# spaceml-org/STARCOP

Measured on AMD Instinct MI355X. Metric: 512x512 hyperspectral tiles/sec (train fwd+bwd), higher is better.
Workload: dtype f32; 1 GPU; configs[1]: HyperSTARCOP U-Net (smp.Unet mobilenet_v2, 4ch mag1c+RGB) train step fwd+loss+bwd+Adam, 512x512 tiles, fp32 HIP kernels (3x3 convs: fp32 operands split exactly into 16-bit terms on the matrix cores, fp32 accumulation; see config.precision and DESIGN.md section 2); batch_per_gpu=16, global_batch=16, parallelism=dp1, hipgraph=False, precision=fp32

## Files before the change

starcop_amd/csrc/conv_mfma.hip:

```cpp
#include "sc_common.h"
#include <vector>
#include <cstdlib>

namespace {

struct ConvP {
  SrcD s0, s1;
  const float* wpk;
  int N, H, W, Cout;
  float* out0; float* out1;
  int csplit, accum0, accum1;
  const float* add0; const float* add1;
  float* stats;
  int xcdmap;
};

template <int KS, int RM, bool BNB, int PF_ = 1>
__global__ __launch_bounds__(256, 2) void k_conv_mfma(const ConvP p) {
  constexpr int TAPS = KS * KS;
  constexpr int CO_T = 32 * RM;
  constexpr int PR = (KS == 3) ? 6 : 4;
  constexpr int PC = (KS == 3) ? 34 : 32;
  constexpr int PCH = PR * PC;
  constexpr int KC = (KS == 3) ? 8 : 16;
// ... 327 lines not shown
  const int lane = tid & 63, wave = tid >> 6;
  const int l15 = lane & 15, lq = lane >> 4;
  const int n = blockIdx.z;
  const int H = p.H, W = p.W;
  const int tiles_x = (W + 31) >> 5;
  const int ty = blockIdx.x / tiles_x;
  const int y0 = ty * 4 * RW, x0 = (blockIdx.x - ty * tiles_x) * 32;
  const int C0 = p.s0.C;
  const int Cin = C0 + p.s1.C;
  const int nk = (Cin + KC - 1) / KC;
  const float* wbase = p.wpk;

  floatx4 acc[RW][2];
#pragma unroll
  for (int rr = 0; rr < RW; ++rr) { acc[rr][0] = (floatx4){0.f, 0.f, 0.f, 0.f}; acc[rr][1] = acc[rr][0]; }

  const int sci = tid >> 5, sq = tid & 31;
  unsigned off0[NE], off1[NE];
  unsigned inb = 0;
  {
    const int up0 = p.s0.up, up1 = p.s1.up;
    const int Ws0 = W >> up0, Ws1 = W >> up1;
#pragma unroll
    for (int i = 0; i < NE; ++i) {
      const int e = sq + 32 * i;
      const int pr = e / PC, pc = e - pr * PC;
      const int y = y0 - 1 + pr, x = x0 - 1 + pc;
      const bool ok = (e < PCH) && (y >= 0) && (y < H) && (x >= 0) && (x < W);
      off0[i] = ok ? (unsigned)((y >> up0) * Ws0 + (x >> up0)) : 0u;
      off1[i] = ok ? (unsigned)((y >> up1) * Ws1 + (x >> up1)) : 0u;
      inb |= ok ? (1u << i) : 0u;
    }
  }
  float xv[NE], av[BNB ? NE : 1];
  float4 c0 = make_float4(1.f, 0.f, 0.f, 0.f);
  float c4 = 0.f, slo = 0.f, shi = 0.f;
  bool chok = true;
  floatx4 wv[NW];

  auto load_chunk = [&](int kc) {
    const int cg = kc * KC + sci;
    const bool second = cg >= C0;
    const SrcD& s = second ? p.s1 : p.s0;
    chok = cg < Cin;
    const int cs = chok ? (second ? cg - C0 : cg) : 0;
    slo = sc_act_lo(s.act); shi = sc_act_hi(s.act);
    if (s.mode != SC_SRC_RAW) { c0 = *reinterpret_cast<const float4*>(s.cst + (size_t)cs * SC_CST); c4 = BNB ? s.cst[(size_t)cs * SC_CST + 4] : 0.f; }
    else { c0 = make_float4(1.f, 0.f, 0.f, 0.f); c4 = 0.f; }
    const size_t plane = (size_t)(H >> s.up) * (W >> s.up);
    const float* xb = s.x + ((size_t)n * s.C + cs) * plane;
    const float* ab = BNB ? s.aux + ((size_t)n * s.C + cs) * plane : nullptr;
#pragma unroll
    for (int i = 0; i < NE; ++i) {
      const unsigned o = second ? off1[i] : off0[i];
      xv[i] = xb[o];
      if (BNB) av[i] = ab[o];
    }
    const floatx4* wsrc = reinterpret_cast<const floatx4*>(wbase + (size_t)kc * WCH);
#pragma unroll
    for (int j = 0; j < NW; ++j) {
      const int i4 = tid + 256 * j;
      wv[j] = wsrc[i4 < WCH / 4 ? i4 : WCH / 4 - 1];
    }
  };
  auto store_chunk = [&](int buf) {
#pragma unroll
    for (int i = 0; i < NE; ++i) {
      const float t = BNB ? sc_pro_bnbwd(xv[i], av[BNB ? i : 0], c0.x, c0.y, c0.z, c0.w, c4, slo, shi) : sc_pro_affine(xv[i], c0.x, c0.y, slo, shi);
      s_p[buf][sci * PCHP + sq + 32 * i] = (((inb >> i) & 1u) && chok) ? t : 0.f;
    }
#pragma unroll
    for (int j = 0; j < NW; ++j) *reinterpret_cast<floatx4*>(&s_w[buf][(tid + 256 * j) * 4]) = wv[j];
  };
  auto compute_chunk = [&](int buf) {
#pragma unroll
    for (int kq = 0; kq < KC / 4; ++kq) {
      const int cil = 4 * kq + lq;
#pragma unroll
      for (int tap = 0; tap < TAPS; ++tap) {
        const int kh = tap / 3, kw = tap - 3 * kh;
        const float a = s_w[buf][(cil * TAPS + tap) * CO_T + l15];
#pragma unroll
        for (int rr = 0; rr < RW; ++rr)
#pragma unroll
          for (int pb = 0; pb < 2; ++pb) {
            const float b = s_p[buf][cil * PCHP + (wave * RW + rr + kh) * PC + pb * 16 + l15 + kw];
            acc[rr][pb] = __builtin_amdgcn_mfma_f32_16x16x4f32(a, b, acc[rr][pb], 0, 0, 0);
          }
      }
    }
  };

  load_chunk(0);
  store_chunk(0);
  __syncthreads();
  for (int kc = 0; kc < nk; ++kc) {
    const bool more = (kc + 1) < nk;
    if (more) load_chunk(kc + 1);
    compute_chunk(kc & 1);
    if (more) store_chunk((kc + 1) & 1);
    __syncthreads();
  }

  const size_t HWs = (size_t)H * W;
  const bool want_stats = p.stats != nullptr;
#pragma unroll
  for (int r = 0; r < 4; ++r) {
    const int co = 4 * lq + r;
    float s = 0.f, ss = 0.f;
#pragma unroll
    for (int rr = 0; rr < RW; ++rr) {
      const int oy = y0 + wave * RW + rr;
#pragma unroll
      for (int pb = 0; pb < 2; ++pb) {
        const int ox = x0 + pb * 16 + l15;
        float v = acc[rr][pb][r];
        const bool ok = (oy < H) && (ox < W) && (co < p.Cout);
        if (!ok) v = 0.f;
        s += v; ss = fmaf(v, v, ss);
        if (ok) {
          const size_t idx = ((size_t)n * p.Cout + co) * HWs + (size_t)oy * W + ox;
          if (p.add0) v += p.add0[idx];
          if (p.add1) v += p.add1[idx];
          if (p.accum0) v += p.out0[idx];
          p.out0[idx] = v;
        }
      }
    }
    if (want_stats) {
      SC_DPP_ADD(s, 0xB1, 0xF); SC_DPP_ADD(s, 0x4E, 0xF); SC_DPP_ADD(s, 0x141, 0xF); SC_DPP_ADD(s, 0x140, 0xF);
      SC_DPP_ADD(ss, 0xB1, 0xF); SC_DPP_ADD(ss, 0x4E, 0xF); SC_DPP_ADD(ss, 0x141, 0xF); SC_DPP_ADD(ss, 0x140, 0xF);
      if (l15 == 0) { s_red[wave][co][0] = s; s_red[wave][co][1] = ss; }
    }
  }
  if (want_stats) {
    __syncthreads();
    const int rows4 = (H + 3) >> 2;
    const int tx = blockIdx.x - ty * tiles_x;
    for (int i = tid; i < RW * CO_T * 2; i += 256) {
      const int hh = i / (CO_T * 2), rem = i - hh * (CO_T * 2);
      const int co = rem >> 1, k2 = rem & 1;
      const int t4 = RW * ty + hh;
      if (co < p.Cout && t4 < rows4) {
        float t = 0.f;
#pragma unroll
        for (int w2 = 0; w2 < 4 / RW; ++w2) t += s_red[hh * (4 / RW) + w2][co][k2];
        const size_t row = ((size_t)n * rows4 + t4) * tiles_x + tx;
        p.stats[(row * p.Cout + co) * 2 + k2] = t;
      }
    }
  }
}

template <int RM, bool BNB>
__global__ __launch_bounds__(256, 2) void k_conv1_ksplit(const ConvP p) {
  constexpr int CO_T = 32 * RM, KC = 16, PS = 33;
  __shared__ float s_acc[4][CO_T * PS];
  const int tid = threadIdx.x, lane = tid & 63, wave = tid >> 6;
  const int l31 = lane & 31, lhi = lane >> 5;
  const int n = blockIdx.z, cot = blockIdx.y;
  const int HW = p.H * p.W;
  const int p0 = blockIdx.x * 32;
  const int Cin = p.s0.C;
  const int nk = (Cin + KC - 1) / KC;
  const float* wbase = p.wpk + (size_t)cot * nk * KC * CO_T;
  const int pix = p0 + l31;
  const bool pok = pix < HW;
  const float* xb = p.s0.x + (size_t)n * Cin * HW + (pok ? pix : 0);
  const float* ab = BNB ? p.s0.aux + (size_t)n * Cin * HW + (pok ? pix : 0) : nullptr;
  const float* cst = p.s0.cst;
  const float lo = sc_act_lo(p.s0.act), hi = sc_act_hi(p.s0.act);

  floatx16 acc[RM];
#pragma unroll
  for (int m = 0; m < RM; ++m)
#pragma unroll
    for (int r = 0; r < 16; ++r) acc[m][r] = 0.f;

  float bx[8], by[BNB ? 8 : 1], wa[8][RM];
  float4 c0[8]; float c4[BNB ? 8 : 1];
  auto load_chunk = [&](int kc) {
#pragma unroll
    for (int cp = 0; cp < 8; ++cp) {
      const int ci = kc * KC + 2 * cp + lhi;
      const int cc = ci < Cin ? ci : 0;
      bx[cp] = xb[(size_t)cc * HW];
      if (BNB) by[cp] = ab[(size_t)cc * HW];
      if (BNB) { c0[cp] = *reinterpret_cast<const float4*>(cst + (size_t)cc * SC_CST); c4[cp] = cst[(size_t)cc * SC_CST + 4]; }
      else { const float2 t = *reinterpret_cast<const float2*>(cst + (size_t)cc * SC_CST); c0[cp] = make_float4(t.x, t.y, 0.f, 0.f); }
#pragma unroll
      for (int m = 0; m < RM; ++m) wa[cp][m] = wbase[(size_t)ci * CO_T + m * 32 + l31];
    }
  };
  int kc = wave;
  if (kc < nk) load_chunk(kc);
  while (kc < nk) {
    float b[8], a[8][RM];
#pragma unroll
    for (int cp = 0; cp < 8; ++cp) {
      const int ci = kc * KC + 2 * cp + lhi;
      const float t = BNB ? sc_pro_bnbwd(bx[cp], by[BNB ? cp : 0], c0[cp].x, c0[cp].y, c0[cp].z, c0[cp].w, c4[BNB ? cp : 0], lo, hi)
                          : sc_pro_affine(bx[cp], c0[cp].x, c0[cp].y, lo, hi);
      b[cp] = (pok && ci < Cin) ? t : 0.f;
#pragma unroll
      for (int m = 0; m < RM; ++m) a[cp][m] = wa[cp][m];
    }
    const int kn = kc + 4;
    load_chunk(kn < nk ? kn : kc);
#pragma unroll
    for (int cp = 0; cp < 8; ++cp)
#pragma unroll
      for (int m = 0; m < RM; ++m) acc[m] = __builtin_amdgcn_mfma_f32_32x32x2f32(a[cp][m], b[cp], acc[m], 0, 0, 0);
    kc = kn;
  }
#pragma unroll
  for (int m = 0; m < RM; ++m)
#pragma unroll
    for (int r = 0; r < 16; ++r) s_acc[wave][(m * 32 + (r & 3) + 8 * (r >> 2) + 4 * lhi) * PS + l31] = acc[m][r];
  __syncthreads();
  const int px = tid & 31, cg = tid >> 5;
  const int opix = p0 + px;
  const bool ok_px = opix < HW;
  const size_t HWs = (size_t)HW;
  const size_t srow = (size_t)n * gridDim.x + blockIdx.x;
  const bool single = p.csplit == p.Cout;
  const size_t cbase = ((size_t)n * p.Cout + (size_t)cot * CO_T) * HWs;
  float* const ob = p.out0 + cbase;
  const float* const a0 = p.add0 ? p.add0 + cbase : nullptr;
  const float* const a1 = p.add1 ? p.add1 + cbase : nullptr;
#pragma unroll
  for (int i = 0; i < CO_T / 8; ++i) {
    const int col = cg + 8 * i;
    const int co = cot * CO_T + col;
    float v = s_acc[0][col * PS + px] + s_acc[1][col * PS + px] + s_acc[2][col * PS + px] + s_acc[3][col * PS + px];
    const bool ok = ok_px && (co < p.Cout);
    if (!ok) v = 0.f;
    if (p.stats) {
      const float s = half_sum32(v), ss = half_sum32(v * v);
      if ((lane & 31) == SC_HALF_SUM_LANE && co < p.Cout) {
        p.stats[(srow * p.Cout + co) * 2] = s;
        p.stats[(srow * p.Cout + co) * 2 + 1] = ss;
      }
    }
    if (ok) {
      if (single) {
        const unsigned off = (unsigned)col * (unsigned)HWs + (unsigned)opix;
        if (a0) v += a0[off];
        if (a1) v += a1[off];
        if (p.accum0) v += ob[off];
        ob[off] = v;
        continue;
      }
      float* o; size_t idx; int accum;
      if (co < p.csplit) {
        idx = ((size_t)n * p.csplit + co) * HWs + opix; o = p.out0; accum = p.accum0;
      } else {
        idx = ((size_t)n * (p.Cout - p.csplit) + (co - p.csplit)) * HWs + opix; o = p.out1; accum = p.accum1;
      }
      if (p.add0) v += p.add0[idx];
      if (p.add1) v += p.add1[idx];
      if (accum) v += o[idx];
      o[idx] = v;
    }
  }
}

#ifndef SC_PWS_PD
#define SC_PWS_PD 8
#endif
struct PwsP {
  const float* x; const float* aux; const float* cst; int act;
  const float* wpk; int co_t, Kpad;
  float* out; float* stats;
  int HW, K, M;
};

template <int NCB, int NKS, int CP, bool BNB = false>
__global__ __launch_bounds__(256) void k_pw_stream(const PwsP p) {
  constexpr int PD = NKS < SC_PWS_PD ? NKS : SC_PWS_PD;
  constexpr int NPG = 4 / CP;
  constexpr int CW = BNB ? 8 : 2;
  __shared__ __attribute__((aligned(16))) float s_cst[NKS * 4 * CW];
  __shared__ float s_red[4][NCB * 16][2];
  const int tid = threadIdx.x, lane = tid & 63, wave = __builtin_amdgcn_readfirstlane(tid >> 6);
  const int n16 = lane & 15, kq = lane >> 4;
  const int K = p.K, M = p.M, HW = p.HW;
  for (int c = tid; c < NKS * 4; c += 256) {
    if constexpr (BNB) {
      float4 c0 = make_float4(1.f, 0.f, 0.f, 0.f); float c4 = 0.f;
      if (c < K) { c0 = *reinterpret_cast<const float4*>(p.cst + (size_t)c * SC_CST); c4 = p.cst[(size_t)c * SC_CST + 4]; }
      *reinterpret_cast<float4*>(&s_cst[8 * c]) = c0;
      *reinterpret_cast<float4*>(&s_cst[8 * c + 4]) = make_float4(c4, 0.f, 0.f, 0.f);
    } else {
      float sc = 1.f, sh = 0.f;
      if (c < K && p.cst != nullptr) { sc = p.cst[(size_t)c * SC_CST]; sh = p.cst[(size_t)c * SC_CST + 1]; }
      s_cst[2 * c] = sc; s_cst[2 * c + 1] = sh;
    }
  }
  const int pg = wave % NPG, part = wave / NPG;
  const long gpx = ((long)blockIdx.x * NPG + pg) * 64;
  const int img = (int)(gpx / HW), px0 = (int)(gpx - (long)img * HW) + 4 * n16;
  const float* xb = p.x + (size_t)img * K * HW + px0;
  const float* yb = BNB ? p.aux + (size_t)img * K * HW + px0 : nullptr;
  float4 xr[PD], yr[BNB ? PD : 1];
#pragma unroll
  for (int u = 0; u < PD; ++u) {
    const int k = 4 * u + kq;
    xr[u] = *reinterpret_cast<const float4*>(xb + (size_t)(k < K ? k : 0) * HW);
    if constexpr (BNB) yr[u] = *reinterpret_cast<const float4*>(yb + (size_t)(k < K ? k : 0) * HW);
  }
  float A[NCB][NKS];
#pragma unroll
  for (int cb = 0; cb < NCB; ++cb) {
    const int m = (part * NCB + cb) * 16 + n16;
    const float* wp = p.wpk + ((size_t)(m / p.co_t) * p.Kpad) * p.co_t + (m % p.co_t);
#pragma unroll
    for (int ks = 0; ks < NKS; ++ks) {
      const int k = 4 * ks + kq;
      A[cb][ks] = (m < M && k < K) ? wp[(size_t)k * p.co_t] : 0.f;
    }
  }
  floatx4 acc[NCB][4];
#pragma unroll
  for (int cb = 0; cb < NCB; ++cb)
#pragma unroll
    for (int j = 0; j < 4; ++j) acc[cb][j] = (floatx4){0.f, 0.f, 0.f, 0.f};
  const float lo = sc_act_lo(p.act), hi = sc_act_hi(p.act);
  __syncthreads();
#pragma unroll
  for (int ks = 0; ks < NKS; ++ks) {
    const float4 v = xr[ks % PD];
    float4 y = make_float4(0.f, 0.f, 0.f, 0.f);
    if constexpr (BNB) y = yr[ks % PD];
    if (ks + PD < NKS) {
      const int k = 4 * (ks + PD) + kq;
      xr[ks % PD] = *reinterpret_cast<const float4*>(xb + (size_t)(k < K ? k : 0) * HW);
      if constexpr (BNB) yr[ks % PD] = *reinterpret_cast<const float4*>(yb + (size_t)(k < K ? k : 0) * HW);
    }
    float b[4];
    if constexpr (BNB) {
      const float4 c = *reinterpret_cast<const float4*>(&s_cst[8 * (4 * ks + kq)]);
      const float c4 = s_cst[8 * (4 * ks + kq) + 4];
      b[0] = sc_pro_bnbwd(v.x, y.x, c.x, c.y, c.z, c.w, c4, lo, hi); b[1] = sc_pro_bnbwd(v.y, y.y, c.x, c.y, c.z, c.w, c4, lo, hi);
      b[2] = sc_pro_bnbwd(v.z, y.z, c.x, c.y, c.z, c.w, c4, lo, hi); b[3] = sc_pro_bnbwd(v.w, y.w, c.x, c.y, c.z, c.w, c4, lo, hi);
    } else {
      const float2 c = *reinterpret_cast<const float2*>(&s_cst[2 * (4 * ks + kq)]);
      b[0] = sc_pro_affine(v.x, c.x, c.y, lo, hi); b[1] = sc_pro_affine(v.y, c.x, c.y, lo, hi);
      b[2] = sc_pro_affine(v.z, c.x, c.y, lo, hi); b[3] = sc_pro_affine(v.w, c.x, c.y, lo, hi);
    }
#pragma unroll
    for (int cb = 0; cb < NCB; ++cb)
#pragma unroll
      for (int j = 0; j < 4; ++j) acc[cb][j] = __builtin_amdgcn_mfma_f32_16x16x4f32(A[cb][ks], b[j], acc[cb][j], 0, 0, 0);
  }
  float* ob = p.out + (size_t)img * M * HW + px0;
  const bool want_stats = p.stats != nullptr;
#pragma unroll
  for (int cb = 0; cb < NCB; ++cb)
#pragma unroll
    for (int r = 0; r < 4; ++r) {
      const int col = cb * 16 + 4 * kq + r, co = part * NCB * 16 + col;
      const float4 o = make_float4(acc[cb][0][r], acc[cb][1][r], acc[cb][2][r], acc[cb][3][r]);
      if (co < M) *reinterpret_cast<float4*>(ob + (size_t)co * HW) = o;
      if (want_stats) {
        float sv = (o.x + o.y) + (o.z + o.w), sq = fmaf(o.x, o.x, fmaf(o.y, o.y, fmaf(o.z, o.z, o.w * o.w)));
        sv = row_sum16(sv); sq = row_sum16(sq);
        if (n16 == 0) { s_red[wave][col][0] = sv; s_red[wave][col][1] = sq; }
// ... 555 lines not shown
    if (hipMalloc(&d, h.size() * sizeof(float)) != hipSuccess) return nullptr;
    if (hipMemcpy(d, h.data(), h.size() * sizeof(float), hipMemcpyHostToDevice) != hipSuccess) { (void)hipFree(d); return nullptr; }
    table[dev] = d;
  }
  return table[dev];
}

const float* sc_identity_cst_table(int C) { return sc_identity_cst(C); }

extern "C" int sc_pw_stream_variant(const sc_conv_args* a) {
  if (a == nullptr || a->ks != 1 || a->nsrc != 1 || a->N <= 0 || a->H <= 0 || a->W <= 0 || a->Cout <= 0) return -1;
  if (a->co_t != 32 && a->co_t != 64) return -1;
  static const bool pws_off = [] { const char* e = getenv("STARCOP_PWS"); return e && atoi(e) == 0; }();
  const long HWl = (long)a->H * a->W;
  const int K = a->src[0].C, M = a->Cout;
  if (K <= 0 || K % 8 != 0) return -1;
  const bool bnb = a->src[0].mode == SC_SRC_BNBWD;
  if (a->src[0].mode != SC_SRC_RAW && a->src[0].cst == nullptr) return -1;
  if (bnb && a->src[0].aux == nullptr) return -1;
  const bool plain = (a->src[0].mode == SC_SRC_RAW || a->src[0].mode == SC_SRC_AFFINE || (bnb && a->bnr == nullptr && a->stats == nullptr)) &&
                     a->src[0].up == 0 && a->csplit == a->Cout && !a->accum0 && a->add0 == nullptr && a->add1 == nullptr && a->out0 != nullptr;
  const bool aligned = (((uintptr_t)a->src[0].x | (uintptr_t)a->out0 | (bnb ? (uintptr_t)a->src[0].aux : 0)) & 15) == 0;
  const int nks = K / 4;
  const bool ks_ok = bnb ? (nks == 4 || nks == 6 || nks == 8) : (nks == 6 || nks == 8);
  if (pws_off || !plain || !aligned || !ks_ok || M > 192 || HWl < 4096 || HWl % 256 != 0 || HWl >= (1L << 30)) return -1;
  const int ncb = bnb ? (M <= 32 ? 2 : (M <= 96 ? 3 : (M <= 160 ? 5 : 6))) : (M <= 16 ? 1 : (M <= 32 ? 2 : (M <= 160 ? 5 : 6)));
  return (bnb ? 100 : 0) + 10 * ncb + nks;
}

extern "C" int sc_conv2d_mfma(const sc_conv_args* a, sc_stream stream) {
  SC_REQUIRE(a != nullptr, "sc_conv2d_mfma: null args");
  SC_REQUIRE(a->ks == 1 || a->ks == 3, "sc_conv2d_mfma: ks must be 1 or 3 (got %d)", a->ks);
  SC_REQUIRE(a->co_t == 16 || a->co_t == 32 || a->co_t == 64, "sc_conv2d_mfma: co_t must be 16, 32 or 64 (got %d)", a->co_t);
  SC_REQUIRE(a->co_t != 16 || (a->ks == 3 && a->Cout <= 16 && a->csplit == a->Cout),
             "sc_conv2d_mfma: co_t=16 is the thin-layer kernel: ks=3, Cout<=16, single output");
  SC_REQUIRE(a->nsrc == 1 || a->nsrc == 2, "sc_conv2d_mfma: nsrc must be 1 or 2");
  const int C0 = a->src[0].C, C1 = a->nsrc == 2 ? a->src[1].C : 0;
  SC_REQUIRE(C0 > 0 && C0 % 8 == 0 && C1 % 8 == 0, "sc_conv2d_mfma: source channels must be multiples of 8 (got %d,%d)", C0, C1);
  SC_REQUIRE(a->nsrc == 1 || a->ks == 3, "sc_conv2d_mfma: a channel concat of two sources needs ks=3");
  SC_REQUIRE(a->N > 0 && a->H > 0 && a->W > 0 && a->Cout > 0, "sc_conv2d_mfma: bad shape");
  SC_REQUIRE(a->csplit > 0 && a->csplit <= a->Cout, "sc_conv2d_mfma: bad csplit");
  SC_REQUIRE(a->csplit == a->Cout || (a->add0 == nullptr && a->add1 == nullptr), "sc_conv2d_mfma: add tensors need a single output");
  for (int s = 0; s < a->nsrc; ++s) {
    SC_REQUIRE(a->src[s].up == 0 || (a->ks == 3 && a->H % 2 == 0 && a->W % 2 == 0), "sc_conv2d_mfma: upsampled source needs ks=3 and even H,W");
    SC_REQUIRE(a->src[s].mode == SC_SRC_RAW || a->src[s].cst != nullptr, "sc_conv2d_mfma: source %d needs constants", s);
    SC_REQUIRE(a->src[s].mode != SC_SRC_BNBWD || a->src[s].aux != nullptr, "sc_conv2d_mfma: BNBWD source needs aux");
    SC_REQUIRE(a->src[s].mode != SC_SRC_BNBWD || a->nsrc == 1, "sc_conv2d_mfma: a BNBWD source cannot be part of a concat");
  }
  const int pws = a->ks == 1 ? sc_pw_stream_variant(a) : -1;
  if (a->ks == 1) {
    const long HWl = (long)a->H * a->W;
    const int K = a->src[0].C, M = a->Cout;
    if (pws >= 0) {
      const bool bnb = pws >= 100;
      const int ncb = (pws / 10) % 10, nks = pws % 10;
      PwsP q;
      q.x = a->src[0].x; q.aux = a->src[0].aux; q.cst = a->src[0].mode == SC_SRC_RAW ? nullptr : a->src[0].cst;
      q.act = a->src[0].mode == SC_SRC_RAW ? (int)SC_ACT_NONE : a->src[0].act;
      q.wpk = a->wpk; q.co_t = a->co_t; q.Kpad = (K + 15) / 16 * 16;
      q.out = a->out0; q.stats = a->stats; q.HW = (int)HWl; q.K = K; q.M = M;
      hipStream_t st = (hipStream_t)stream;
      const long groups = (long)a->N * HWl / 64;
#define SC_PWS(NCB_, NKS_, CP_) hipLaunchKernelGGL((k_pw_stream<NCB_, NKS_, CP_>), dim3((unsigned)(groups / (4 / CP_))), dim3(256), 0, st, q)
#define SC_PWS_K(NCB_, CP_) do { if (nks == 6) SC_PWS(NCB_, 6, CP_); else SC_PWS(NCB_, 8, CP_); } while (0)
      if (bnb) {
#define SC_PWSB(NCB_, CP_) do { if (nks == 4) hipLaunchKernelGGL((k_pw_stream<NCB_, 4, CP_, true>), dim3((unsigned)(groups / (4 / CP_))), dim3(256), 0, st, q); \
                                else if (nks == 6) hipLaunchKernelGGL((k_pw_stream<NCB_, 6, CP_, true>), dim3((unsigned)(groups / (4 / CP_))), dim3(256), 0, st, q); \
                                else hipLaunchKernelGGL((k_pw_stream<NCB_, 8, CP_, true>), dim3((unsigned)(groups / (4 / CP_))), dim3(256), 0, st, q); } while (0)
        if (ncb == 2) SC_PWSB(2, 1);
        else if (ncb == 3) SC_PWSB(3, 2);
        else if (ncb == 5) SC_PWSB(5, 2);
        else SC_PWSB(6, 2);
#undef SC_PWSB
      }
      else if (ncb == 1) SC_PWS_K(1, 1);
      else if (ncb == 2) SC_PWS_K(2, 1);
      else if (ncb == 5) SC_PWS_K(5, 2);
      else SC_PWS_K(6, 2);
#undef SC_PWS_K
#undef SC_PWS
      SC_LAUNCH_OK("sc_conv2d_mfma(k_pw_stream)");
      return SC_OK;
    }
  }
  ConvP p;
  p.s0 = to_srcd(a->src[0]);
  p.s1 = a->nsrc == 2 ? to_srcd(a->src[1]) : empty_srcd();
  if (a->ks == 1) {
    if (p.s0.mode == SC_SRC_RAW) { p.s0.cst = sc_identity_cst(p.s0.C); SC_REQUIRE(p.s0.cst != nullptr, "sc_conv2d_mfma: identity constants unavailable (C = %d)", p.s0.C); }
    if (a->nsrc == 2 && p.s1.mode == SC_SRC_RAW) { p.s1.cst = sc_identity_cst(p.s1.C); SC_REQUIRE(p.s1.cst != nullptr, "sc_conv2d_mfma: identity constants unavailable (C = %d)", p.s1.C); }
  }
  p.wpk = a->wpk; p.N = a->N; p.H = a->H; p.W = a->W; p.Cout = a->Cout;
  p.out0 = a->out0; p.out1 = a->out1; p.csplit = a->csplit; p.accum0 = a->accum0; p.accum1 = a->accum1;
  p.add0 = a->add0; p.add1 = a->add1; p.stats = a->stats;
  const int co_tiles = (a->Cout + a->co_t - 1) / a->co_t;
  dim3 grid;
  if (a->ks == 3) grid = dim3(((a->W + 31) / 32) * ((a->H + 3) / 4), co_tiles, a->N);
  else grid = dim3((a->H * a->W + 127) / 128, co_tiles, a->N);
  hipStream_t st = (hipStream_t)stream;
  p.xcdmap = 0;
  constexpr int xcdmap_env = 0;
  if (a->co_t != 16 && xcdmap_env) {
    const long total = (long)grid.x * a->N, per_xcd = (total + 7) / 8;
    SC_REQUIRE(per_xcd * 8 * co_tiles < (1L << 31), "sc_conv2d_mfma: grid too large");
    grid = dim3((unsigned)(per_xcd * 8 * co_tiles));
    p.xcdmap = 1;
  }
  if (a->co_t == 16) {
    const bool bnb = a->src[0].mode == SC_SRC_BNBWD;
    if (a->H >= 8) {
      dim3 g2(((a->W + 31) / 32) * ((a->H + 7) / 8), 1, a->N);
      if (bnb) hipLaunchKernelGGL((k_conv_mfma16<true, 2>), g2, dim3(256), 0, st, p);
      else hipLaunchKernelGGL((k_conv_mfma16<false, 2>), g2, dim3(256), 0, st, p);
    } else {
      if (bnb) hipLaunchKernelGGL((k_conv_mfma16<true, 1>), grid, dim3(256), 0, st, p);
      else hipLaunchKernelGGL((k_conv_mfma16<false, 1>), grid, dim3(256), 0, st, p);
    }
  }
  else {
    const bool bnb = a->src[0].mode == SC_SRC_BNBWD;
#define SC_CM(KS_, RM_)                                                                               \
    do {                                                                                              \
      if (bnb) hipLaunchKernelGGL((k_conv_mfma<KS_, RM_, true>), grid, dim3(256), 0, st, p);          \
      else hipLaunchKernelGGL((k_conv_mfma<KS_, RM_, false>), grid, dim3(256), 0, st, p);             \
    } while (0)
    constexpr int pf_env = 1;
#define SC_CM2(RM_)                                                                                  \
    do {                                                                                              \
      if (bnb) hipLaunchKernelGGL((k_conv_mfma<1, RM_, true, 2>), grid, dim3(256), 0, st, p);         \
      else hipLaunchKernelGGL((k_conv_mfma<1, RM_, false, 2>), grid, dim3(256), 0, st, p);            \
    } while (0)
    if (a->ks == 3 && a->co_t == 64) SC_CM(3, 2);
    else if (a->ks == 3) SC_CM(3, 1);
    else if (a->co_t == 64) { if (pf_env == 2) SC_CM2(2); else SC_CM(1, 2); }
    else { if (pf_env == 2) SC_CM2(1); else SC_CM(1, 1); }
#undef SC_CM2
#undef SC_CM
  }
  SC_LAUNCH_OK("sc_conv2d_mfma");
  return SC_OK;
}

extern "C" int sc_conv1x1_ksplit(const sc_conv_args* a, sc_stream stream) {
  SC_REQUIRE(a != nullptr, "sc_conv1x1_ksplit: null args");
  SC_REQUIRE(a->ks == 1 && a->nsrc == 1, "sc_conv1x1_ksplit: ks must be 1 with a single source");
  SC_REQUIRE(a->co_t == 32 || a->co_t == 64, "sc_conv1x1_ksplit: co_t must be 32 or 64 (got %d)", a->co_t);
  SC_REQUIRE(a->src[0].C > 0 && a->src[0].up == 0, "sc_conv1x1_ksplit: bad source");
  SC_REQUIRE(a->src[0].mode != SC_SRC_NORM, "sc_conv1x1_ksplit: NORM sources are the stem's");
  SC_REQUIRE(a->src[0].mode == SC_SRC_RAW || a->src[0].cst != nullptr, "sc_conv1x1_ksplit: source needs constants");
  SC_REQUIRE(a->src[0].mode != SC_SRC_BNBWD || a->src[0].aux != nullptr, "sc_conv1x1_ksplit: BNBWD source needs aux");
  SC_REQUIRE(a->N > 0 && a->H > 0 && a->W > 0 && a->Cout > 0, "sc_conv1x1_ksplit: bad shape");
  SC_REQUIRE(a->csplit > 0 && a->csplit <= a->Cout, "sc_conv1x1_ksplit: bad csplit");
  SC_REQUIRE(a->csplit == a->Cout || (a->add0 == nullptr && a->add1 == nullptr), "sc_conv1x1_ksplit: add tensors need a single output");
  ConvP p;
  p.xcdmap = 0;
  p.s0 = to_srcd(a->src[0]); p.s1 = empty_srcd();
  if (p.s0.mode == SC_SRC_RAW) { p.s0.cst = sc_identity_cst(p.s0.C); SC_REQUIRE(p.s0.cst != nullptr, "sc_conv1x1_ksplit: identity constants unavailable (C = %d)", p.s0.C); }
  p.wpk = a->wpk; p.N = a->N; p.H = a->H; p.W = a->W; p.Cout = a->Cout;
  p.out0 = a->out0; p.out1 = a->out1; p.csplit = a->csplit; p.accum0 = a->accum0; p.accum1 = a->accum1;
  p.add0 = a->add0; p.add1 = a->add1; p.stats = a->stats;
  dim3 grid((a->H * a->W + 31) / 32, (a->Cout + a->co_t - 1) / a->co_t, a->N);
  hipStream_t st = (hipStream_t)stream;
  const bool bnb = a->src[0].mode == SC_SRC_BNBWD;
  if (a->co_t == 64 && bnb) hipLaunchKernelGGL((k_conv1_ksplit<2, true>), grid, dim3(256), 0, st, p);
  else if (a->co_t == 64) hipLaunchKernelGGL((k_conv1_ksplit<2, false>), grid, dim3(256), 0, st, p);
  else if (bnb) hipLaunchKernelGGL((k_conv1_ksplit<1, true>), grid, dim3(256), 0, st, p);
  else hipLaunchKernelGGL((k_conv1_ksplit<1, false>), grid, dim3(256), 0, st, p);
  SC_LAUNCH_OK("sc_conv1x1_ksplit");
  return SC_OK;
}

extern "C" size_t sc_wgrad_workspace_floats(int N, int H, int W, int Cout, int Cin, int ks) {
  const WgradPlan pl = plan_wgrad(N, H, W, Cout, Cin, ks);
  const size_t E = (size_t)ks * ks * pl.CoP * pl.CiP;
  const int nparts = pl.nsl * (ks == 1 ? 1 : pl.wk);
  return (size_t)nparts * E + sc_reduce_scratch_floats(nparts, E);
}

static int wgrad_mfma_launch(const sc_wgrad_args* a, sc_stream stream, sc_wgrad_pending* pending);

extern "C" int sc_conv2d_wgrad_mfma(const sc_wgrad_args* a, sc_stream stream) { return wgrad_mfma_launch(a, stream, nullptr); }

extern "C" int sc_conv2d_wgrad_mfma_deferred(const sc_wgrad_args* a, sc_wgrad_pending* pending, sc_stream stream) {
  SC_REQUIRE(pending != nullptr, "sc_conv2d_wgrad_mfma_deferred: null descriptor");
  return wgrad_mfma_launch(a, stream, pending);
}

static int wgrad_mfma_launch(const sc_wgrad_args* a, sc_stream stream, sc_wgrad_pending* pending) {
  SC_REQUIRE(a != nullptr, "sc_conv2d_wgrad_mfma: null args");
  SC_REQUIRE(a->ks == 1 || a->ks == 3, "sc_conv2d_wgrad_mfma: ks must be 1 or 3");
  SC_REQUIRE(a->nsrc == 1 || a->nsrc == 2, "sc_conv2d_wgrad_mfma: nsrc must be 1 or 2");
  const int C0 = a->src[0].C, C1 = a->nsrc == 2 ? a->src[1].C : 0;
  SC_REQUIRE(C0 + C1 == a->Cin, "sc_conv2d_wgrad_mfma: source channels (%d+%d) != Cin %d", C0, C1, a->Cin);
  SC_REQUIRE(a->dy.C == a->Cout, "sc_conv2d_wgrad_mfma: dy channels %d != Cout %d", a->dy.C, a->Cout);
  SC_REQUIRE(a->dy.up == 0, "sc_conv2d_wgrad_mfma: dy cannot be upsampled");
  SC_REQUIRE(a->dy.mode != SC_SRC_BNBWD || a->dy.aux != nullptr, "sc_conv2d_wgrad_mfma: BNBWD dy needs aux");
  for (int s = 0; s < a->nsrc; ++s) {
    SC_REQUIRE(a->src[s].mode != SC_SRC_BNBWD, "sc_conv2d_wgrad_mfma: input sources cannot be BNBWD");
    SC_REQUIRE(a->src[s].up == 0 || (a->ks == 3 && a->H % 2 == 0 && a->W % 2 == 0), "sc_conv2d_wgrad_mfma: upsampled source needs ks=3, even H,W");
  }
  const WgradPlan pl = plan_wgrad(a->N, a->H, a->W, a->Cout, a->Cin, a->ks);
  SC_REQUIRE(pl.stages < (1L << 31), "sc_conv2d_wgrad_mfma: too many stages (%ld) for the kernel's 32-bit stage arithmetic", pl.stages);
  const size_t need = sc_wgrad_workspace_floats(a->N, a->H, a->W, a->Cout, a->Cin, a->ks);
  SC_REQUIRE(a->part_floats >= need, "sc_conv2d_wgrad_mfma: workspace too small (%zu < %zu floats)", a->part_floats, need);
  WgradP p;
  p.dy = to_srcd(a->dy); p.s0 = to_srcd(a->src[0]); p.s1 = a->nsrc == 2 ? to_srcd(a->src[1]) : empty_srcd();
  p.N = a->N; p.H = a->H; p.W = a->W; p.Cout = a->Cout; p.Cin = a->Cin; p.part = a->part;
  p.nsl = pl.nsl; p.CoP = pl.CoP; p.CiP = pl.CiP;
  dim3 grid(pl.nsl, pl.ci_tiles, pl.co_tiles);
  hipStream_t st = (hipStream_t)stream;
#define SC_WG(KS, WM, WN) hipLaunchKernelGGL((k_wgrad_mfma<KS, WM, WN>), grid, dim3(256), 0, st, p)
  if (pl.wm == 0) {
    if (pl.wn == 2) hipLaunchKernelGGL((k_wgrad_mfma16<2>), grid, dim3(256), 0, st, p);
    else hipLaunchKernelGGL((k_wgrad_mfma16<1>), grid, dim3(256), 0, st, p);
  } else if (a->ks == 3) {
    if (pl.wm == 2 && pl.wn == 2) SC_WG(3, 2, 2);
    else if (pl.wm == 2) SC_WG(3, 2, 1);
    else if (pl.wn == 2) SC_WG(3, 1, 2);
    else SC_WG(3, 1, 1);
  } else {
    if (pl.wm == 2 && pl.wn == 2) SC_WG(1, 2, 2);
    else if (pl.wm == 2) SC_WG(1, 2, 1);
    else if (pl.wn == 2) SC_WG(1, 1, 2);
    else SC_WG(1, 1, 1);
  }
#undef SC_WG
  SC_LAUNCH_OK("sc_conv2d_wgrad_mfma");
  if (pending) {
    pending->part = a->part; pending->dw = a->dw;
    pending->nparts = pl.nsl * (a->ks == 1 ? 1 : pl.wk); pending->taps = a->ks * a->ks;
    pending->Cout = a->Cout; pending->Cin = a->Cin; pending->CoP = pl.CoP; pending->CiP = pl.CiP;
    pending->total = (uint64_t)pending->taps * a->Cout * a->Cin;
    return SC_OK;
  }
  return sc_wgrad_finish(a->part, pl.nsl * (a->ks == 1 ? 1 : pl.wk), a->ks * a->ks, a->Cout, a->Cin, pl.CoP, pl.CiP, a->dw, st);
}

namespace {
__global__ __launch_bounds__(256) void k_wgrad_reduce_batch(const sc_wgrad_pending* __restrict__ descs, const unsigned* __restrict__ starts, int n) {
  int lo = 0, hi = n - 1;
  while (lo < hi) {
    const int mid = (lo + hi + 1) >> 1;
    if (starts[mid] <= blockIdx.x) lo = mid; else hi = mid - 1;
  }
  const sc_wgrad_pending d = descs[lo];
  const size_t i = (size_t)(blockIdx.x - starts[lo]) * 256 + threadIdx.x;
  if (i >= d.total) return;
  const int ci = (int)(i % d.Cin);
  size_t r = i / d.Cin;
  const int co = (int)(r % d.Cout);
  const int tap = (int)(r / d.Cout);
  const size_t plane = (size_t)d.CoP * d.CiP, stride = (size_t)d.taps * plane;
  const float* src = d.part + (size_t)tap * plane + (size_t)co * d.CiP + ci;
  float s = 0.f;
  int k = 0;
  for (; k + 8 <= d.nparts; k += 8) {
    float v[8];
#pragma unroll
    for (int u = 0; u < 8; ++u) v[u] = src[(size_t)(k + u) * stride];
#pragma unroll
    for (int u = 0; u < 8; ++u) s += v[u];
  }
  for (; k < d.nparts; ++k) s += src[(size_t)k * stride];
  d.dw[((size_t)co * d.Cin + ci) * d.taps + tap] = s;
}
}

extern "C" int sc_wgrad_reduce_batch(const sc_wgrad_pending* descs_dev, const uint32_t* block_starts_dev, int n, uint32_t total_blocks,
                                     sc_stream stream) {
  SC_REQUIRE(descs_dev && block_starts_dev && n >= 0, "sc_wgrad_reduce_batch: bad argument");
  if (n == 0 || total_blocks == 0) return SC_OK;
  hipLaunchKernelGGL(k_wgrad_reduce_batch, dim3(total_blocks), dim3(256), 0, (hipStream_t)stream, descs_dev, block_starts_dev, n);
  SC_LAUNCH_OK("sc_wgrad_reduce_batch");
  return SC_OK;
}

int sc_wgrad_finish(float* part, int nparts, int taps, int Cout, int Cin, int CoP, int CiP, float* dw, hipStream_t st) {
  const size_t E = (size_t)taps * CoP * CiP;
  const float* rows; int nrows;
  int rc = sc_reduce_rows_partial(part, nparts, E, part + (size_t)nparts * E, &rows, &nrows, 64, st);
  if (rc != SC_OK) return rc;
  const size_t total = (size_t)taps * Cout * Cin;
  const int blocks = (int)((total + 255) / 256 > 4096 ? 4096 : (total + 255) / 256);
  hipLaunchKernelGGL(k_wgrad_reduce, dim3(blocks), dim3(256), 0, st, rows, dw, nrows, taps, Cout, Cin, CoP, CiP);
  SC_LAUNCH_OK("sc_wgrad_reduce");
  return SC_OK;
}
```

Before: 1436 tiles/s.

## Deepen 1x1 k-split conv load pipeline and stage per-channel constants in LDS

Restructures the 1x1 k-split conv kernel into an explicit multi-slot software pipeline (2 or 3 chunks in flight) with scheduling barriers. Per-channel affine/BN constants are staged once into LDS instead of being reloaded per chunk. Address math moves to 32-bit byte offsets with immediate offsets. Occupancy hint rises to 4 blocks per CU and shared memory becomes dynamic. This hides global-load latency and cuts redundant constant loads, at the cost of more registers (spill risk at the higher occupancy target) and a new 2^30-element size limit.

```diff
diff --git a/starcop_amd/csrc/conv_mfma.hip b/starcop_amd/csrc/conv_mfma.hip
--- a/starcop_amd/csrc/conv_mfma.hip
+++ b/starcop_amd/csrc/conv_mfma.hip
@@ -503,11 +503,17 @@
   }
 }
 
+__device__ __forceinline__ float sc_ld_off(const float* base, unsigned byte_off, int imm) {
+  return *reinterpret_cast<const float*>(reinterpret_cast<const char*>(base) + (size_t)byte_off + imm);
+}
+
 template <int RM, bool BNB>
-__global__ __launch_bounds__(256, 2) void k_conv1_ksplit(const ConvP p) {
+__global__ __launch_bounds__(256, 4) void k_conv1_ksplit(const ConvP p) {
   constexpr int CO_T = 32 * RM, KC = 16, PS = 33;
-  __shared__ float s_acc[4][CO_T * PS];
-  const int tid = threadIdx.x, lane = tid & 63, wave = tid >> 6;
+  constexpr int D = (RM == 1 && !BNB) ? 3 : 2;
+  extern __shared__ __attribute__((aligned(16))) float s_dyn[];
+  float (*s_acc)[CO_T * PS] = reinterpret_cast<float (*)[CO_T * PS]>(s_dyn);
+  const int tid = threadIdx.x, lane = tid & 63, wave = __builtin_amdgcn_readfirstlane(tid >> 6);
   const int l31 = lane & 31, lhi = lane >> 5;
   const int n = blockIdx.z, cot = blockIdx.y;
   const int HW = p.H * p.W;
@@ -517,53 +523,102 @@
   const float* wbase = p.wpk + (size_t)cot * nk * KC * CO_T;
   const int pix = p0 + l31;
   const bool pok = pix < HW;
-  const float* xb = p.s0.x + (size_t)n * Cin * HW + (pok ? pix : 0);
-  const float* ab = BNB ? p.s0.aux + (size_t)n * Cin * HW + (pok ? pix : 0) : nullptr;
+  const float* xn = p.s0.x + (size_t)n * Cin * HW;
+  const float* an = BNB ? p.s0.aux + (size_t)n * Cin * HW : nullptr;
   const float* cst = p.s0.cst;
   const float lo = sc_act_lo(p.s0.act), hi = sc_act_hi(p.s0.act);
 
+  for (int c = tid; c < nk * KC; c += 256) {
+    const int q = (c & ~15) | ((c & 1) << 3) | ((c & 15) >> 1);
+    if (BNB) {
+      float4 c0 = make_float4(0.f, 0.f, 0.f, 0.f); float c4 = 0.f;
+      if (c < Cin) { c0 = *reinterpret_cast<const float4*>(cst + (size_t)c * SC_CST); c4 = cst[(size_t)c * SC_CST + 4]; }
+      *reinterpret_cast<float4*>(s_dyn + q * 4) = c0;
+      s_dyn[nk * KC * 4 + q] = c4;
+    } else {
+      float2 c0 = make_float2(0.f, 0.f);
+      if (c < Cin) c0 = *reinterpret_cast<const float2*>(cst + (size_t)c * SC_CST);
+      *reinterpret_cast<float2*>(s_dyn + q * 2) = c0;
+    }
+  }
+  __syncthreads();
+
   floatx16 acc[RM];
 #pragma unroll
   for (int m = 0; m < RM; ++m)
 #pragma unroll
     for (int r = 0; r < 16; ++r) acc[m][r] = 0.f;
 
-  float bx[8], by[BNB ? 8 : 1], wa[8][RM];
-  float4 c0[8]; float c4[BNB ? 8 : 1];
-  auto load_chunk = [&](int kc) {
-#pragma unroll
-    for (int cp = 0; cp < 8; ++cp) {
-      const int ci = kc * KC + 2 * cp + lhi;
-      const int cc = ci < Cin ? ci : 0;
-      bx[cp] = xb[(size_t)cc * HW];
-      if (BNB) by[cp] = ab[(size_t)cc * HW];
-      if (BNB) { c0[cp] = *reinterpret_cast<const float4*>(cst + (size_t)cc * SC_CST); c4[cp] = cst[(size_t)cc * SC_CST + 4]; }
-      else { const float2 t = *reinterpret_cast<const float2*>(cst + (size_t)cc * SC_CST); c0[cp] = make_float4(t.x, t.y, 0.f, 0.f); }
-#pragma unroll
-      for (int m = 0; m < RM; ++m) wa[cp][m] = wbase[(size_t)ci * CO_T + m * 32 + l31];
-    }
-  };
-  int kc = wave;
-  if (kc < nk) load_chunk(kc);
-  while (kc < nk) {
-    float b[8], a[8][RM];
-#pragma unroll
-    for (int cp = 0; cp < 8; ++cp) {
-      const int ci = kc * KC + 2 * cp + lhi;
-      const float t = BNB ? sc_pro_bnbwd(bx[cp], by[BNB ? cp : 0], c0[cp].x, c0[cp].y, c0[cp].z, c0[cp].w, c4[BNB ? cp : 0], lo, hi)
-                          : sc_pro_affine(bx[cp], c0[cp].x, c0[cp].y, lo, hi);
-      b[cp] = (pok && ci < Cin) ? t : 0.f;
-#pragma unroll
-      for (int m = 0; m < RM; ++m) a[cp][m] = wa[cp][m];
-    }
-    const int kn = kc + 4;
-    load_chunk(kn < nk ? kn : kc);
-#pragma unroll
-    for (int cp = 0; cp < 8; ++cp)
-#pragma unroll
-      for (int m = 0; m < RM; ++m) acc[m] = __builtin_amdgcn_mfma_f32_32x32x2f32(a[cp][m], b[cp], acc[m], 0, 0, 0);
-    kc = kn;
-  }
+  const int nw = (nk - wave + 3) >> 2;
+  const unsigned xpix = (unsigned)(pok ? pix : 0) * 4u;
+  const unsigned xch = (unsigned)HW * 4u;
+  const unsigned xlane = xpix + (unsigned)lhi * xch;
+  const unsigned wlane = (unsigned)(lhi * CO_T + l31) * 4u;
+  float bx[D][8], by[BNB ? D : 1][8], wa[D][8][RM];
+
+#define KSP_ISSUE(slot, j_)                                                                        \
+  {                                                                                                \
+    const int kk_ = min(wave + 4 * (j_), nk - 1);                                                  \
+    const int cb_ = kk_ * KC + lhi;                                                                \
+    unsigned xo_ = xlane + (unsigned)(kk_ * KC) * xch;              \
+    unsigned wo_ = wlane + (unsigned)kk_ * (unsigned)(KC * CO_T * 4);                              \
+    asm volatile("" : "+v"(xo_), "+v"(wo_));           \
+    _Pragma("unroll") for (int cp = 0; cp < 8; ++cp) {                                             \
+      const unsigned o_ = cb_ + 2 * cp < Cin ? xo_ + (unsigned)(2 * cp) * xch : xpix;              \
+      bx[slot][cp] = sc_ld_off(xn, o_, 0);                                                         \
+      if (BNB) by[BNB ? slot : 0][cp] = sc_ld_off(an, o_, 0);                                      \
+    }                                                                                              \
+    _Pragma("unroll") for (int cp = 0; cp < 8; ++cp)                                               \
+      _Pragma("unroll") for (int m = 0; m < RM; ++m)                                               \
+        wa[slot][cp][m] = sc_ld_off(wbase, wo_, (2 * cp * CO_T + m * 32) * 4);      \
+    __builtin_amdgcn_sched_barrier(0);                                                             \
+  }
+
+#define KSP_CONSUME(slot, j_)                                                                      \
+  {                                                                                                \
+    int cb_ = (wave + 4 * (j_)) * KC + lhi * 8;                     \
+    asm volatile("" : "+v"(cb_));                      \
+    const int ci0_ = (wave + 4 * (j_)) * KC + lhi;                                                 \
+    float b[8];                                                                                    \
+    if (BNB) {                                                                                     \
+      const float4* q0 = reinterpret_cast<const float4*>(s_dyn + cb_ * 4);                         \
+      const float* q4 = s_dyn + nk * KC * 4 + cb_;                                                 \
+      _Pragma("unroll") for (int cp = 0; cp < 8; ++cp) {                                           \
+        const float4 c0 = q0[cp];                                                                  \
+        const float t = sc_pro_bnbwd(bx[slot][cp], by[BNB ? slot : 0][cp], c0.x, c0.y, c0.z, c0.w, q4[cp], lo, hi); \
+        b[cp] = (pok && ci0_ + 2 * cp < Cin) ? t : 0.f;                                            \
+      }                                                                                            \
+    } else {                                                                                       \
+      const float2* q0 = reinterpret_cast<const float2*>(s_dyn + cb_ * 2);                         \
+      _Pragma("unroll") for (int cp = 0; cp < 8; ++cp) {                                           \
+        const float2 c0 = q0[cp];                                                                  \
+        const float t = sc_pro_affine(bx[slot][cp], c0.x, c0.y, lo, hi);                           \
+        b[cp] = (pok && ci0_ + 2 * cp < Cin) ? t : 0.f;                                            \
+      }                                                                                            \
+    }                                                                                              \
+    _Pragma("unroll") for (int cp = 0; cp < 8; ++cp)                                               \
+      _Pragma("unroll") for (int m = 0; m < RM; ++m)                                               \
+        acc[m] = __builtin_amdgcn_mfma_f32_32x32x2f32(wa[slot][cp][m], b[cp], acc[m], 0, 0, 0);    \
+    _Pragma("unroll") for (int m = 0; m < RM; ++m) asm volatile("" : "+v"(acc[m]));                \
+    __builtin_amdgcn_sched_barrier(0);                                                             \
+  }
+
+#pragma unroll
+  for (int s = 0; s < D; ++s) KSP_ISSUE(s, s)
+  int j0 = 0;
+  for (; j0 + D <= nw; j0 += D) {
+#pragma unroll
+    for (int s = 0; s < D; ++s) {
+      KSP_CONSUME(s, j0 + s)
+      KSP_ISSUE(s, j0 + s + D)
+    }
+  }
+#pragma unroll
+  for (int s = 0; s < D - 1; ++s)
+    if (j0 + s < nw) KSP_CONSUME(s, j0 + s)
+#undef KSP_CONSUME
+#undef KSP_ISSUE
+  __syncthreads();
 #pragma unroll
   for (int m = 0; m < RM; ++m)
 #pragma unroll
@@ -1425,6 +1480,8 @@
   SC_REQUIRE(a->N > 0 && a->H > 0 && a->W > 0 && a->Cout > 0, "sc_conv1x1_ksplit: bad shape");
   SC_REQUIRE(a->csplit > 0 && a->csplit <= a->Cout, "sc_conv1x1_ksplit: bad csplit");
   SC_REQUIRE(a->csplit == a->Cout || (a->add0 == nullptr && a->add1 == nullptr), "sc_conv1x1_ksplit: add tensors need a single output");
+  SC_REQUIRE((long long)a->src[0].C * a->H * a->W < (1LL << 30) && (long long)a->Cout * a->H * a->W < (1LL << 30),
+             "sc_conv1x1_ksplit: an image of the source or of the output has 2^30 elements or more");
   ConvP p;
   p.xcdmap = 0;
   p.s0 = to_srcd(a->src[0]); p.s1 = empty_srcd();
@@ -1435,10 +1492,19 @@
   dim3 grid((a->H * a->W + 31) / 32, (a->Cout + a->co_t - 1) / a->co_t, a->N);
   hipStream_t st = (hipStream_t)stream;
   const bool bnb = a->src[0].mode == SC_SRC_BNBWD;
-  if (a->co_t == 64 && bnb) hipLaunchKernelGGL((k_conv1_ksplit<2, true>), grid, dim3(256), 0, st, p);
-  else if (a->co_t == 64) hipLaunchKernelGGL((k_conv1_ksplit<2, false>), grid, dim3(256), 0, st, p);
-  else if (bnb) hipLaunchKernelGGL((k_conv1_ksplit<1, true>), grid, dim3(256), 0, st, p);
-  else hipLaunchKernelGGL((k_conv1_ksplit<1, false>), grid, dim3(256), 0, st, p);
+  const size_t kp = (size_t)((a->src[0].C + 15) / 16) * 16;
+  const size_t lds_acc = (size_t)4 * a->co_t * 33 * sizeof(float), lds_cst = kp * (bnb ? 5 : 2) * sizeof(float);
+  const size_t lds = lds_acc > lds_cst ? lds_acc : lds_cst;
+#define SC_KSP(RM_, BNB_)                                                                          \
+  do {                                                                                             \
+    if (int rc = sc_lds_limit(k_conv1_ksplit<RM_, BNB_>, lds, "sc_conv1x1_ksplit")) return rc;     \
+    hipLaunchKernelGGL((k_conv1_ksplit<RM_, BNB_>), grid, dim3(256), lds, st, p);                  \
+  } while (0)
+  if (a->co_t == 64 && bnb) SC_KSP(2, true);
+  else if (a->co_t == 64) SC_KSP(2, false);
+  else if (bnb) SC_KSP(1, true);
+  else SC_KSP(1, false);
+#undef SC_KSP
   SC_LAUNCH_OK("sc_conv1x1_ksplit");
   return SC_OK;
 }
```

Result: faster. 1453 tiles/s, median of 6 (+1.2%).
